# openshift/kubernetes-autoscaler

Hardware: NVIDIA B200
Metric: pod x node predicate evals/sec (higher is better)
Workload: dtype int64

## Files before the change

kubernetes-autoscaler_b200/csrc/api.cu:

```cuda
#include <algorithm>
#include <chrono>
#include <cstdio>
#include <cstdlib>
#include <cstring>
#include <map>
#include <tuple>
#include <unordered_map>

#include "engine.h"

namespace cae {

static thread_local std::string g_err;
void set_error(const std::string& msg) { g_err = msg; }

int Arena::alloc(void** dev, void** stage, size_t bytes) {
  bytes = (std::max<size_t>(bytes, 16) + 255) & ~(size_t)255;
  for (;;) {
    if (cur < chunks.size() && chunks[cur].used + bytes <= chunks[cur].size) break;
    if (cur + 1 < chunks.size()) { ++cur; continue; }
    Chunk c;
    c.size = std::max(bytes, min_chunk);
    if (cudaMalloc(&c.dev, c.size) != cudaSuccess) { set_error("cudaMalloc failed"); return -1; }
    if (mirrored && cudaHostAlloc(&c.host, c.size, cudaHostAllocDefault) != cudaSuccess) { set_error("cudaHostAlloc failed"); return -1; }
// ... 146 lines not shown
  UPV(dom, d.dom); UPV(dc_spec, d.dc_spec); UPV(dc_sc, d.dc_sc); UPV(dc_q_off, d.dc_q_off); UPV(q_kind, d.q_kind);
  UPV(q_k, d.q_k); UPV(q_dc, d.q_dc); UPV(q_p0, d.q_p0); UPV(q_base_off, d.q_base_off);
  UPV(spec_used, p8); e->d_spec_used = p8;
  UPV(dc_ngroups, p32); e->d_dc_ngroups = p32;
#undef UPV
  const size_t Q = std::max(d.Q, 1), pool = std::max(q_base_off.back(), 1);
  if (dev_alloc(e, &d.wmat, Q * S) || dev_alloc(e, &d.q_self, Q) || dev_alloc(e, &d.q_wown, Q) || dev_alloc(e, &d.q_active, Q) ||
      dev_alloc(e, &d.dc_aff_self, (size_t)d.DC) || dev_alloc(e, &d.dc_active, (size_t)d.DC) || dev_alloc(e, &d.elig, Q * e->U) ||
      dev_alloc(e, &d.base_cnt, pool, true) || dev_alloc(e, &d.base_pres, pool, true) || dev_alloc(e, &d.base_tot, Q, true) ||
      dev_alloc(e, &d.ds_w, Q * std::max(T, 1)) || dev_alloc(e, &d.st_min1, Q) || dev_alloc(e, &d.st_arg1, Q) ||
      dev_alloc(e, &d.st_min2, Q) || dev_alloc(e, &d.st_ndom, Q) || dev_alloc(e, &d.st_nmin, Q) || dev_alloc(e, &d.q_nfeed, Q, true) ||
      dev_alloc(e, &d.group_feeds, (size_t)std::max(e->E, 1), true) || dev_alloc(e, &d.qrec, Q))
    return -1;
  e->h_dc_of_spec_valid = true;
  return 0;
}

struct LoadTimer {
  bool on;
  std::chrono::steady_clock::time_point t0;
  std::string out;
  LoadTimer() : on(getenv("CAE_LOAD_TIMING") != nullptr), t0(std::chrono::steady_clock::now()) {}
  void mark(const char* what) {
    if (!on) return;
    auto t1 = std::chrono::steady_clock::now();
    char buf[96];
    snprintf(buf, sizeof(buf), " %s=%.1fus", what, std::chrono::duration<double, std::micro>(t1 - t0).count());
    out += buf;
    t0 = t1;
  }
  ~LoadTimer() { if (on) fprintf(stderr, "cae_load:%s\n", out.c_str()); }
};

static int stage_pending(Engine* e, int P, const int32_t* pend_spec, int E, const int32_t* group_off, bool check_pending) {
  const size_t words = (size_t)P + E + 1;
  if (words > e->pending_stage_words) {
    if (e->h_pending_stage) cudaFreeHost(e->h_pending_stage);
    e->h_pending_stage = nullptr;
    e->pending_stage_words = 0;
    const size_t cap_words = std::max(words, (size_t)e->cap_P + e->cap_E + 1);
    CAE_CUDA(cudaHostAlloc(reinterpret_cast<void**>(&e->h_pending_stage), cap_words * 4, cudaHostAllocDefault));
    e->pending_stage_words = cap_words;
  }
  const int S = e->num_podspecs;
  std::vector<int32_t> gspec(E, -1);
  bool homog = true;
  for (int g = 0; g < E; ++g) {
    const int b = group_off[g], en = group_off[g + 1];
    if (en <= b) continue;
    const int s0 = pend_spec[b];
    if (check_pending && (s0 < 0 || s0 >= S || !e->h_spec_pending[s0])) { set_error("cae_load_pending: a pod spec that was not pending at the last cae_load"); return 2; }
    gspec[g] = s0;
    int diff = 0;
    for (int p = b + 1; p < en; ++p) diff |= pend_spec[p] ^ s0;
    homog &= diff == 0;
  }
  if (!homog && check_pending)
    for (int p = 0; p < P; ++p) {
      const int s = pend_spec[p];
      if (s < 0 || s >= S || !e->h_spec_pending[s]) { set_error("cae_load_pending: a pod spec that was not pending at the last cae_load"); return 2; }
    }
  if (P) memcpy(e->h_pending_stage, pend_spec, sizeof(int32_t) * P);
  memcpy(e->h_pending_stage + P, group_off, sizeof(int32_t) * (E + 1));
  e->h_pend_spec = e->h_pending_stage;
  e->h_group_off = e->h_pending_stage + P;
  e->h_group_spec.swap(gspec);
  e->groups_homogeneous = homog;
  return 0;
}

static int do_load(Engine* e, const cae_objects* o) {
  LoadTimer lt;
  if (o->abi_version != CAE_ABI_VERSION) { set_error("cae_objects.abi_version mismatch"); return -2; }
  if (o->num_res < 3 || o->num_res > CAE_MAX_RES) { set_error("num_res out of range"); return 1; }
  e->up.reset();
  e->scratch.reset();
  e->loaded = false;
  e->group_reason_valid = false;
  e->stats.h2d_bytes = 0;
  const int N = o->num_cluster_nodes, T = o->num_templates, NT = N + T;
  e->N = N; e->T = T; e->U = N + 2 * T; e->E = o->num_groups; e->P = o->num_pending;
  e->Tw = (T + 31) / 32;
  e->Twp = (e->Tw + FEAS_TW - 1) / FEAS_TW * FEAS_TW;
  e->num_podspecs = o->num_podspecs;
  const int W = std::max(1, e->cfg.world_size), rk = e->cfg.rank;
  e->p_begin = (int)((int64_t)e->P * rk / W);
  e->p_end = (int)((int64_t)e->P * (rk + 1) / W);
  e->p_begin = (e->p_begin / 32) * 32;
  if (rk + 1 < W) e->p_end = (e->p_end / 32) * 32;
  if (e->cfg.flags & CAE_CFG_PODS_PRESHARDED) { e->p_begin = 0; e->p_end = e->P; }
  e->Pl = e->p_end - e->p_begin;
  e->Plw = (e->Pl + 31) / 32;
  e->t_begin = (int)((int64_t)T * rk / W);
  e->t_end = (int)((int64_t)T * (rk + 1) / W);

  cudaEventRecord(e->ev0, e->stream);
  DevObjects& d = e->dobj;
  d.num_res = o->num_res; d.num_values = o->num_values; d.hostname_key = o->hostname_key;
  d.unschedulable_taint_key = o->unschedulable_taint_key; d.N = N; d.T = T;
  UP(value_is_int, o->num_values); UP(value_int, o->num_values);
// ... 129 lines not shown
    }
  }
  e->feas_B = 0;
  e->feas_fstart = 0;
  for (int a = 0; a < e->A; ++a) {
    const int nb = f_bits[a] - 1;
    for (int i = nb - 1; i >= 0; --i) {
      if (e->feas_B >= 32) { set_error("resource request cardinality too large for the bit-sliced encoding"); return 1; }
      e->feas_sword[e->feas_B] = (uint8_t)f_word[a];
      e->feas_sshift[e->feas_B] = (uint8_t)(f_shift[a] + i);
      if (i == nb - 1) e->feas_fstart |= 1u << e->feas_B;
      ++e->feas_B;
    }
  }
  e->lut_rows = 0;
  for (int a = 0; a < e->A; ++a) {
    e->lut_base[a] = e->lut_rows;
    e->lut_rows += (int)rvals[a].size() + 1;
    e->lut_word[a] = (uint8_t)f_word[a];
    e->lut_shift[a] = (uint8_t)f_shift[a];
    e->lut_mask[a] = (1u << (f_bits[a] - 1)) - 1u;
  }
  e->d_tslice = nullptr;
  if (e->force_bitslice || e->lut_rows > FEAS_LUT_MAX_ROWS) {
    const int Bpad = std::max(4, (e->feas_B + 3) / 4 * 4);
    std::vector<uint32_t> tslice((size_t)Bpad * std::max(e->Tw, 1), 0);
    for (int b = 0; b < e->feas_B; ++b)
      for (int t = 0; t < T; ++t)
        tslice[(size_t)b * e->Tw + t / 32] |= ((tmpl_w[(size_t)e->feas_sword[b] * T + t] >> e->feas_sshift[b]) & 1u) << (t % 32);
    if (upload_mut(e, tslice, &e->d_tslice)) return -1;
  }
  {
    std::vector<uint32_t> rlut((size_t)std::max(e->lut_rows, 1) * std::max(e->Twp, 1), 0);
    for (int a = 0; a < e->A; ++a)
      for (int t = 0; t < T; ++t) {
        const uint32_t rank_free = (tmpl_w[(size_t)f_word[a] * T + t] >> f_shift[a]) & e->lut_mask[a];
        for (uint32_t k = 0; k <= rank_free; ++k) rlut[(size_t)(e->lut_base[a] + k) * e->Twp + t / 32] |= 1u << (t % 32);
      }
    if (upload_mut(e, rlut, &e->d_rlut)) return -1;
  }
  if (upload_mut(e, spec_sc, &e->d_spec_sc) || upload_mut(e, slots, &e->d_tmpl_slots) ||
      upload_mut(e, free_all, &e->d_tmpl_free_all) || upload_mut(e, free_act, &e->d_tmpl_free) || upload_mut(e, cfree, &e->d_c_free) ||
      upload_mut(e, cslots, &e->d_c_slots) || upload_mut(e, spec_w, &e->d_spec_w) || upload_mut(e, tmpl_w, &e->d_tmpl_w) || upload_mut(e, spec_dc, &e->d_spec_dc))
    return -1;

  lt.mark("ranks+tables");
  if (dev_alloc(e, &e->d_pre_ok, (size_t)e->SC * std::max(e->Twp, 1)) ||
      dev_alloc(e, &e->d_post_code, (size_t)e->DC * std::max(T, 1), true) || dev_alloc(e, &e->d_post_ok, (size_t)e->DC * std::max(e->Twp, 1)) ||
      dev_alloc(e, &e->d_pod_w, (size_t)std::max(e->W, 1) * std::max(e->Pl, 1)) || dev_alloc(e, &e->d_pod_row, (size_t)std::max(e->A, 1) * std::max(e->Pl, 1)) || dev_alloc(e, &e->d_pod_sc, (size_t)std::max(e->Pl, 1)) ||
      dev_alloc(e, &e->d_pod_dc, (size_t)std::max(e->Pl, 1)) || dev_alloc(e, &e->d_fit_bits, (size_t)std::max(T, 1) * std::max(e->Plw, 1)) ||
      dev_alloc(e, &e->d_fit_count, (size_t)std::max(T, 1), true) || dev_alloc(e, &e->d_fit_acc, (size_t)std::max(T, 1), true) ||
      dev_alloc(e, &e->d_chunk_done, (size_t)std::max(e->Twp / FEAS_TW, 1), true) || dev_alloc(e, &e->d_group_reason, (size_t)std::max(T, 1) * std::max(e->E, 1)) ||
      dev_alloc(e, &e->d_counts2, (size_t)2 * std::max(T, 1), true) || dev_alloc(e, &e->d_sched, (size_t)std::max(T, 1) * std::max(e->E, 1), true) ||
      dev_alloc(e, &e->d_order, (size_t)std::max(T, 1) * std::max(e->E, 1)) || dev_alloc(e, &e->d_grec, (size_t)std::max(e->E, 1)) || dev_alloc(e, &e->d_order_n, (size_t)std::max(T, 1), true) ||
      dev_alloc(e, &e->d_max_nodes, (size_t)std::max(T, 1), true) || dev_alloc(e, &e->d_last_index_buf, (size_t)2 * std::max(T, 1), true) || dev_alloc(e, &e->d_tmpl_cost, (size_t)std::max(T, 1), true) ||
      dev_alloc(e, &e->d_perm, (size_t)std::max(T, 1)) || dev_alloc(e, &e->d_work_counter, 4, true) ||
      dev_alloc(e, &e->d_act_dim, CAE_MAX_RES))
    return -1;
  e->d_score = nullptr;
  e->d_reasons = nullptr;
  if (e->cfg.want_reasons && dev_alloc(e, &e->d_reasons, (size_t)std::max(T, 1) * std::max(e->Pl, 1))) return -1;

  e->h_spec_pending = spec_pending;
  e->cap_P = e->P; e->cap_E = e->E; e->cap_Pl = e->Pl;
  { int rc = stage_pending(e, e->P, o->pend_spec, e->E, o->group_off, false); if (rc) return rc; }

  lt.mark("dev_alloc+memsets");
  if (e->up.flush(e->stream, &e->stats.h2d_bytes)) return -1;
  CAE_CUDA(cudaMemcpyAsync(e->d_act_dim, e->act_dim, sizeof(int) * CAE_MAX_RES, cudaMemcpyHostToDevice, e->stream));
  if (launch_pre_ok_bits(e)) return -1;
  if (e->has_dynamic) {
    if (launch_dynamic_tables(e, e->d_spec_used, e->d_dc_ngroups)) return -1;
    std::vector<uint8_t> act(e->dyn.DC);
    CAE_CUDA(cudaMemcpyAsync(act.data(), e->dyn.dc_active, act.size(), cudaMemcpyDeviceToHost, e->stream));
    CAE_CUDA(cudaStreamSynchronize(e->stream));
    bool changed = false;
    for (int s = 0; s < S; ++s) if (spec_dc[s] && !act[spec_dc[s]]) { spec_dc[s] = 0; changed = true; }
    if (changed) CAE_CUDA(cudaMemcpyAsync(e->d_spec_dc, spec_dc.data(), sizeof(int32_t) * S, cudaMemcpyHostToDevice, e->stream));
    e->h_spec_dc = spec_dc;
    CAE_CUDA(cudaStreamSynchronize(e->stream));
  }
  if (launch_post_bits(e)) return -1;
  if (launch_expand_pods(e)) return -1;
  if (launch_group_records(e)) return -1;
  cudaEventRecord(e->ev1, e->stream);
  lt.mark("launches");
  CAE_CUDA(cudaStreamSynchronize(e->stream));
  lt.mark("sync");
  float ms = 0;
  cudaEventElapsedTime(&ms, e->ev0, e->ev1);
  e->stats.h2d_ms = ms;
  e->loaded = true;
  return 0;
}

}

using cae::Engine;
// ... 107 lines not shown
  delete e;
}

int32_t cae_load(cae_engine* h, const cae_objects* objs) {
  if (!h || !objs) return -2;
  Engine* e = reinterpret_cast<Engine*>(h);
  cudaSetDevice(e->cfg.device);
  return cae::do_load(e, objs);
}

int32_t cae_load_pending(cae_engine* h, int32_t num_pending, const int32_t* pend_spec, int32_t num_groups, const int32_t* group_off) {
  Engine* e = reinterpret_cast<Engine*>(h);
  if (!e || !e->loaded) { cae::set_error("cae_load_pending before cae_load"); return -2; }
  if (num_pending < 0 || num_groups < 0 || (num_pending && !pend_spec) || !group_off) { cae::set_error("cae_load_pending: bad arguments"); return -2; }
  cudaSetDevice(e->cfg.device);
  const int P = num_pending, E = num_groups;
  const int W = std::max(1, e->cfg.world_size), rk = e->cfg.rank;
  int pb = (int)((int64_t)P * rk / W), pe = (int)((int64_t)P * (rk + 1) / W);
  pb = (pb / 32) * 32;
  if (rk + 1 < W) pe = (pe / 32) * 32;
  if (e->cfg.flags & CAE_CFG_PODS_PRESHARDED) { pb = 0; pe = P; }
  const int Pl = pe - pb;
  if (P > e->cap_P || E > e->cap_E || Pl > e->cap_Pl) { cae::set_error("cae_load_pending: more pods / groups than the resident buffers hold"); return 2; }
  if (group_off[0] != 0 || group_off[E] != P) { cae::set_error("cae_load_pending: group_off does not cover the pending pods"); return -2; }
  if (e->has_dynamic) {
    bool same = E == e->E;
    for (int g = 0; g < E && same; ++g) {
      const int s_new = group_off[g + 1] > group_off[g] ? pend_spec[group_off[g]] : -1;
      same = s_new == e->h_group_spec[g];
    }
    if (!same) { cae::set_error("cae_load_pending: the group -> spec sequence changed under topology counters"); return 2; }
  }
  CAE_CUDA(cudaStreamSynchronize(e->stream));
  { int rc = cae::stage_pending(e, P, pend_spec, E, group_off, true); if (rc) return rc; }
  const size_t words = (size_t)P + E + 1;
  if (P) CAE_CUDA(cudaMemcpyAsync(const_cast<int32_t*>(e->dobj.pend_spec), e->h_pend_spec, sizeof(int32_t) * P, cudaMemcpyHostToDevice, e->stream));
  CAE_CUDA(cudaMemcpyAsync(const_cast<int32_t*>(e->dobj.group_off), e->h_group_off, sizeof(int32_t) * (E + 1), cudaMemcpyHostToDevice, e->stream));
  e->stats.h2d_bytes = (int64_t)words * 4;
  e->P = P; e->E = E; e->p_begin = pb; e->p_end = pe; e->Pl = Pl; e->Plw = (Pl + 31) / 32;
  e->group_reason_valid = false;
  if (cae::launch_expand_pods(e)) return -1;
  if (cae::launch_group_records(e)) return -1;
  return 0;
}

int32_t cae_feasibility(cae_engine* h, uint32_t* fit_bits, uint8_t* reasons, int32_t* fit_count) {
  Engine* e = reinterpret_cast<Engine*>(h);
  if (!e || !e->loaded) { cae::set_error("cae_feasibility before cae_load"); return -2; }
  cudaSetDevice(e->cfg.device);
  bool want_r = e->cfg.want_reasons && e->d_reasons;
  cudaEventRecord(e->ev0, e->stream);
  if (cae::launch_feasibility(e, want_r)) return -1;
  cudaEventRecord(e->ev1, e->stream);
  e->stats.d2h_bytes = 0;
  if (!e->ev2) { cudaEventCreate(&e->ev2); cudaEventCreate(&e->ev3); }
  cudaEvent_t c0 = e->ev2, c1 = e->ev3;
  cudaEventRecord(c0, e->stream);
  if (fit_bits && e->T && e->Plw) {
    CAE_CUDA(cudaMemcpyAsync(fit_bits, e->d_fit_bits, sizeof(uint32_t) * (size_t)e->T * e->Plw, cudaMemcpyDeviceToHost, e->stream));
    e->stats.d2h_bytes += sizeof(uint32_t) * (size_t)e->T * e->Plw;
  }
  if (reasons && want_r && e->T && e->Pl) {
    CAE_CUDA(cudaMemcpyAsync(reasons, e->d_reasons, (size_t)e->T * e->Pl, cudaMemcpyDeviceToHost, e->stream));
    e->stats.d2h_bytes += (size_t)e->T * e->Pl;
  }
  if (fit_count && e->T) {
    CAE_CUDA(cudaMemcpyAsync(fit_count, e->d_fit_count, sizeof(int32_t) * e->T, cudaMemcpyDeviceToHost, e->stream));
// ... 515 lines not shown
```

kubernetes-autoscaler_b200/csrc/engine.h:

```cpp
#pragma once
#include <cuda_runtime.h>

#include <cstdint>
#include <string>
#include <vector>

#include "../../include/caengine.h"
#include "dyn.cuh"
#include "tables.cuh"

namespace cae {

constexpr int FEAS_MAX_W = 4;
constexpr int FEAS_LUT_MAX_ROWS = 1024;
constexpr int FEAS_TW = 16;

void set_error(const std::string& msg);

struct alignas(16) GroupRec {
  int32_t n, spec, sc, dc;
  uint32_t flags;
  int32_t pad[3];
  unsigned long long pconf, pbit;
  int64_t req[CAE_MAX_RES];
  float rinv[CAE_MAX_RES];
};
static_assert(sizeof(GroupRec) == 144, "GroupRec is fetched as nine 16-byte chunks");
enum : uint32_t { GREC_HAS_PORTS = 1u, GREC_FEEDS = 2u, GREC_HOST_SPREAD = 4u };
constexpr int ORDER_NOT_ON_FRESH = 1 << 30;

#define CAE_CUDA(expr)                                                                        \
  do {                                                                                        \
    cudaError_t _e = (expr);                                                                  \
    if (_e != cudaSuccess) {                                                                  \
      cae::set_error(std::string(#expr) + ": " + cudaGetErrorString(_e));                     \
      return -1;                                                                              \
    }                                                                                         \
  } while (0)

#define CAE_KERNEL_OK()                                                                       \
  do {                                                                                        \
    cudaError_t _e = cudaGetLastError();                                                      \
    if (_e != cudaSuccess) {                                                                  \
      cae::set_error(std::string(__func__) + ": " + cudaGetErrorString(_e));                  \
      return -1;                                                                              \
    }                                                                                         \
  } while (0)

// ... 31 lines not shown
  int A = 0;
  int act_dim[CAE_MAX_RES] = {0};
  int SC = 0, DC = 0;
  int Tw = 0;
  int Twp = 0;
  int p_begin = 0, p_end = 0;
  int t_begin = 0, t_end = 0;
  int Pl = 0, Plw = 0;
  bool has_dynamic = false;

  DevObjects dobj{};
  StaticClass* d_sclass = nullptr;
  uint8_t* d_pre_code = nullptr;
  uint32_t* d_pre_ok = nullptr;
  int32_t* d_spec_sc = nullptr;
  int32_t* d_spec_dc = nullptr;
  uint8_t* d_post_code = nullptr;
  uint32_t* d_post_ok = nullptr;
  int W = 0;
  uint32_t feas_guard[4] = {0, 0, 0, 0};
  uint32_t* d_spec_w = nullptr;
  uint32_t* d_pod_w = nullptr;
  uint16_t* d_pod_row = nullptr;
  uint32_t* d_tmpl_w = nullptr;
  int feas_B = 0;
  uint32_t feas_fstart = 0;
  uint8_t feas_sword[32] = {0}, feas_sshift[32] = {0};
  uint32_t* d_tslice = nullptr;
  int lut_rows = 0;
  int lut_base[CAE_MAX_RES] = {0};
  uint8_t lut_word[CAE_MAX_RES] = {0}, lut_shift[CAE_MAX_RES] = {0};
  uint32_t lut_mask[CAE_MAX_RES] = {0};
  uint32_t* d_rlut = nullptr;
  long long* d_tmpl_cost = nullptr;
  int32_t* d_perm = nullptr;
  int k1_warps = 16;
  bool force_bitslice = false;
  int32_t* d_pod_sc = nullptr;
  int32_t* d_pod_dc = nullptr;
  int64_t* d_tmpl_free = nullptr;
  int64_t* d_tmpl_free_all = nullptr;
  int32_t* d_tmpl_slots = nullptr;
  int64_t* d_spec_req_t = nullptr;
  uint32_t* d_fit_bits = nullptr;
  uint8_t* d_reasons = nullptr;
  int32_t* d_fit_count = nullptr;
  int32_t* d_fit_acc = nullptr;
  int32_t* d_chunk_done = nullptr;
  uint8_t* d_group_reason = nullptr;
  bool group_reason_valid = false;
  int32_t* d_counts2 = nullptr;
  int32_t* d_sched = nullptr;
  int32_t* d_order = nullptr;
  int32_t* d_order_n = nullptr;
  GroupRec* d_grec = nullptr;
  double* d_score = nullptr;
  int32_t* d_max_nodes = nullptr;
  int32_t* d_last_index_buf = nullptr;
  const int32_t* d_last_index_in = nullptr;
  int32_t* d_last_index_out = nullptr;
  int32_t* d_pc_of = nullptr;
  unsigned long long* d_port_conf = nullptr;
  int pack_cap = 1 << 30;
  void* d_pack_scratch = nullptr;
  size_t pack_scratch_bytes = 0;
  size_t pack_layout_sig = 0;
// ... 63 lines not shown
```

kubernetes-autoscaler_b200/csrc/feas.cu:

```cuda
#include <algorithm>
#include <climits>

#include "engine.h"

namespace cae {

struct LutLayout {
  int A, rows;
  int base[CAE_MAX_RES];
  uint32_t mask[CAE_MAX_RES];
  uint8_t word[CAE_MAX_RES], shift[CAE_MAX_RES];
};

static LutLayout lut_layout(const Engine* e) {
  LutLayout lay{};
  lay.A = e->A;
  lay.rows = e->lut_rows;
  for (int d = 0; d < e->A; ++d) {
    lay.base[d] = e->lut_base[d]; lay.mask[d] = e->lut_mask[d]; lay.word[d] = e->lut_word[d]; lay.shift[d] = e->lut_shift[d];
  }
  return lay;
}

__global__ void expand_pods_kernel(const int32_t* __restrict__ pend_spec, int p_begin, int Pl, int W, LutLayout lay,
// ... 10 lines not shown
  }
  pod_sc[p] = spec_sc[spec];
  pod_dc[p] = spec_dc[spec];
}

int launch_expand_pods(Engine* e) {
  if (e->Pl == 0) return 0;
  expand_pods_kernel<<<(e->Pl + 255) / 256, 256, 0, e->stream>>>(e->dobj.pend_spec, e->p_begin, e->Pl, e->W, lut_layout(e), e->d_spec_w,
                                                                   e->d_spec_sc, e->d_spec_dc, e->d_pod_w, e->d_pod_row, e->d_pod_sc, e->d_pod_dc);
  e->stats.kernel_launches++;
  CAE_KERNEL_OK();
  return 0;
}

constexpr int K1_TW = FEAS_TW;
constexpr int K1_TCHUNK = K1_TW * 32;
constexpr int K1_LPITCH = K1_TW + 1;

struct PeerPush {
  int world, rank;
  int tag;
  int2* data[8];
  int32_t* done_ctr;
  int32_t* status;
};

struct K1Args {
  int Pl, Plw, T, Tw, Twp, N, U, W;
  int G, gq, gr;
  const uint32_t* pod_w;
  const uint16_t* pod_row;
  const int32_t *pod_sc, *pod_dc;
  const uint32_t *tslice, *rlut;
  const int32_t* tmpl_slots;
  const uint32_t *pre_ok, *post_ok;
  const uint8_t *pre_code, *post_code;
  uint32_t* fit_bits;
  int32_t *fit_count, *fit_acc, *chunk_done;
  uint8_t* reasons;
};

__device__ __forceinline__ int k1_ld_acquire_sys(const int32_t* p) {
  int v;
  asm volatile("ld.acquire.sys.global.s32 %0, [%1];" : "=r"(v) : "l"(p) : "memory");
  return v;
}
__device__ __forceinline__ void k1_red_release_sys(int32_t* p, int v) {
  asm volatile("red.release.sys.global.add.s32 [%0], %1;" ::"l"(p), "r"(v) : "memory");
}
__device__ __forceinline__ void k1_st_volatile_v2(int2* p, int x, int y) {
  asm volatile("st.volatile.global.v2.s32 [%0], {%1, %2};" ::"l"(p), "r"(x), "r"(y) : "memory");
}
__device__ __forceinline__ int2 k1_ld_volatile_v2(const int2* p) {
  int2 v;
  asm volatile("ld.volatile.global.v2.s32 {%0, %1}, [%2];" : "=r"(v.x), "=r"(v.y) : "l"(p) : "memory");
  return v;
}
__device__ __forceinline__ unsigned long long k1_globaltimer() {
  unsigned long long t;
  asm volatile("mov.u64 %0, %%globaltimer;" : "=l"(t));
  return t;
}

__device__ __forceinline__ void k1_finish(const K1Args& a, const PeerPush& pp, const int32_t* s_cnt, int t0, int tid, int nthreads) {
  __shared__ int s_flag;
  for (int i = tid; i < K1_TCHUNK; i += nthreads) {
    const int c = s_cnt[i];
    if (c && t0 + i < a.T) atomicAdd(&a.fit_acc[t0 + i], c);
  }
  __syncthreads();
  if (tid == 0) {
    __threadfence();
    s_flag = atomicAdd(&a.chunk_done[blockIdx.y], 1) == (int)gridDim.x - 1;
  }
  __syncthreads();
  if (!s_flag) return;
  __threadfence();
  for (int i = tid; i < K1_TCHUNK; i += nthreads) {
    const int t = t0 + i;
    if (t < a.T) {
      a.fit_count[t] = __ldcg(&a.fit_acc[t]);
      a.fit_acc[t] = 0;
    }
  }
  if (tid == 0) a.chunk_done[blockIdx.y] = 0;
  if (!pp.world) return;
  __syncthreads();
  if (tid == 0) {
    __threadfence();
    s_flag = atomicAdd(pp.done_ctr, 1) == (int)gridDim.y - 1;
  }
  __syncthreads();
  if (!s_flag) return;
  __threadfence();
  const int tag = pp.tag;
  for (int r = 0; r < pp.world; ++r) {
    int2* dst = pp.data[r] + (size_t)pp.rank * Engine::PEER_CAP;
    for (int t = tid; t < a.T; t += nthreads) k1_st_volatile_v2(dst + t, __ldcg(&a.fit_count[t]), tag);
  }
  const int2* mine = pp.data[pp.rank];
  const unsigned long long t0ns = k1_globaltimer();
  int ok = 1;
  for (int t = tid; t < a.T && ok; t += nthreads) {
    int2 x[Engine::PEER_MAX];
    unsigned pending = 0;
#pragma unroll
    for (int r = 0; r < Engine::PEER_MAX; ++r)
      if (r < pp.world) x[r] = k1_ld_volatile_v2(mine + (size_t)r * Engine::PEER_CAP + t);
#pragma unroll
    for (int r = 0; r < Engine::PEER_MAX; ++r)
      if (r < pp.world && x[r].y != tag) pending |= 1u << r;
    for (int spins = 0; pending; ) {
#pragma unroll
      for (int r = 0; r < Engine::PEER_MAX; ++r)
        if ((pending >> r) & 1u) {
          x[r] = k1_ld_volatile_v2(mine + (size_t)r * Engine::PEER_CAP + t);
          if (x[r].y == tag) pending &= ~(1u << r);
        }
      if (pending && (++spins & 1023) == 0 && k1_globaltimer() - t0ns > 2000000000ull) { ok = 0; break; }
    }
    int v = 0;
#pragma unroll
    for (int r = 0; r < Engine::PEER_MAX; ++r)
      if (r < pp.world) v += x[r].x;
    if (ok) a.fit_count[t] = v;
  }
  if (!ok) atomicExch(pp.status, 1);
  if (tid == 0) *pp.done_ctr = 0;
}

struct TransposeConsts { uint32_t sel16, sel8, amt[3], keep[3]; };

__device__ __forceinline__ uint32_t opaque(uint32_t v) {
  uint32_t r;
  asm volatile("mov.b32 %0, %1;" : "=r"(r) : "r"(v));
  return r;
}

__device__ __forceinline__ TransposeConsts transpose_consts(int lane) {
  TransposeConsts c;
  c.sel16 = opaque((lane & 16) ? 0x3276u : 0x5410u);
  c.sel8 = opaque((lane & 8) ? 0x3715u : 0x6240u);
#pragma unroll
  for (int i = 0; i < 3; ++i) {
    const int s = 4 >> i;
    const uint32_t lowmask = s == 4 ? 0x0F0F0F0Fu : s == 2 ? 0x33333333u : 0x55555555u;
    c.amt[i] = opaque((lane & s) ? (uint32_t)s : (uint32_t)(32 - s));
    c.keep[i] = opaque((lane & s) ? ~lowmask : lowmask);
  }
  return c;
}

__device__ __forceinline__ uint32_t bitselect(uint32_t x, uint32_t y, uint32_t keep) {
  uint32_t r;
  asm("lop3.b32 %0, %1, %2, %3, 0xE4;" : "=r"(r) : "r"(x), "r"(y), "r"(keep));
  return r;
}

__device__ __forceinline__ void warp_transpose32x2(uint32_t& a, uint32_t& b, const TransposeConsts& c) {
  uint32_t ya = __shfl_xor_sync(0xffffffffu, a, 16), yb = __shfl_xor_sync(0xffffffffu, b, 16);
  a = __byte_perm(a, ya, c.sel16);
// ... 82 lines not shown
        const int wglob = tw0 + tw + h;
        const uint32_t fit = h ? fit1 : fit0;
        if (valid && wglob < a.Tw) {
          for (int j = 0; j < 32; ++j) {
            const int t = wglob * 32 + j;
            if (t >= a.T) break;
            uint8_t rs = a.pre_code[(size_t)sc * a.U + a.N + t] & 0x0F;
            if (rs == 0) rs = (!((fit >> j) & 1u) || a.tmpl_slots[t] < 1) ? CAE_R_FIT : a.post_code[(size_t)dc * a.T + t];
            a.reasons[(size_t)t * a.Pl + p] = rs;
          }
        }
      }
    }
    uint32_t c0 = fit0 & cls[tw], c1 = fit1 & cls[tw + 1];
    warp_transpose32x2(c0, c1, tc);
    s_out[warp * PAD + tw * 32 + lane] = c0;
    s_out[warp * PAD + (tw + 1) * 32 + lane] = c1;
    atomicAdd(&s_cnt[tw * 32 + lane], __popc(c0));
    atomicAdd(&s_cnt[(tw + 1) * 32 + lane], __popc(c1));
  }
  __syncthreads();
  if (a.fit_bits) {
    const int wv = tid % NW;
    if (wv < npw) {
      uint32_t* dst = a.fit_bits + (size_t)(t0 + tid / NW) * a.Plw + pwb + wv;
      const uint32_t* src = s_out + wv * PAD + tid / NW;
      const size_t stride = (size_t)32 * a.Plw;
      const int kmax = min(K1_TCHUNK / 32, (a.T - t0 - tid / NW + 31) / 32);
#pragma unroll 4
      for (int k = 0; k < kmax; ++k, dst += stride, src += 32) *dst = *src;
    }
  }
  k1_finish(a, pp, s_cnt, t0, tid, NT);
}

constexpr int K1_THREADS = 256;
constexpr int K1_WARPS = K1_THREADS / 32;
constexpr int K1_PAD = K1_TCHUNK + 4;

struct FeasLayout {
  uint32_t fstart;
  int nb;
  uint8_t sword[32], sshift[32];
};

template <int B, bool REASONS>
__global__ void __launch_bounds__(K1_THREADS)
feasibility_kernel(K1Args a, FeasLayout lay, PeerPush pp) {
  __shared__ uint32_t s_sl[B > 0 ? B : 1][K1_TW];
  __shared__ uint32_t s_out[K1_WARPS][K1_PAD];
  __shared__ int32_t s_cnt[K1_TCHUNK];
  const int tid = threadIdx.x, lane = tid & 31, warp = tid >> 5;
  const int p = blockIdx.x * K1_THREADS + tid;
  const int tw0 = blockIdx.y * K1_TW;
  const int t0 = tw0 * 32;

  for (int i = tid; i < B * K1_TW; i += K1_THREADS) {
    const int b = i / K1_TW, w = i % K1_TW;
    s_sl[b][w] = (tw0 + w < a.Tw) ? a.tslice[(size_t)b * a.Tw + tw0 + w] : 0u;
  }
  for (int i = tid; i < K1_TCHUNK; i += K1_THREADS) s_cnt[i] = 0;
  const bool valid = p < a.Pl;
  uint32_t r[B > 0 ? B : 1];
  {
    uint32_t pw[FEAS_MAX_W];
#pragma unroll
// ... 40 lines not shown
  }
  __syncthreads();
  const int pw0 = blockIdx.x * K1_WARPS;
  for (int i = tid; i < K1_TCHUNK * K1_WARPS; i += K1_THREADS) {
    const int tl = i / K1_WARPS, wv = i % K1_WARPS;
    const int t = t0 + tl;
    if (t < a.T && pw0 + wv < a.Plw && a.fit_bits) a.fit_bits[(size_t)t * a.Plw + pw0 + wv] = s_out[wv][tl];
  }
  k1_finish(a, pp, s_cnt, t0, tid, K1_THREADS);
}

static PeerPush peer_push_args(Engine* e) {
  PeerPush pp{};
  if (e->peer_world > 1 && e->T <= Engine::PEER_CAP) {
    const int par = (int)(e->peer_step & 1);
    const size_t blk = (size_t)Engine::PEER_MAX * Engine::PEER_CAP;
    pp.world = e->peer_world;
    pp.rank = e->cfg.rank;
    e->peer_step += 1;
    pp.tag = (int)(e->peer_step & 0x7fffffff);
    if (pp.tag == 0) pp.tag = 1;
    for (int r = 0; r < e->peer_world; ++r) pp.data[r] = reinterpret_cast<int2*>(e->peer_base[r]) + par * blk;
    pp.done_ctr = e->d_xbuf + 4 * blk + 8;
    pp.status = e->d_xbuf + 4 * blk + 9;
  }
  return pp;
}

static K1Args k1_args(Engine* e) {
  K1Args a{};
  a.Pl = e->Pl; a.Plw = e->Plw; a.T = e->T; a.Tw = e->Tw; a.Twp = e->Twp; a.N = e->N; a.U = e->U; a.W = e->W;
  a.G = 1;
  a.pod_w = e->d_pod_w; a.pod_row = e->d_pod_row; a.pod_sc = e->d_pod_sc; a.pod_dc = e->d_pod_dc;
  a.tslice = e->d_tslice; a.rlut = e->d_rlut; a.tmpl_slots = e->d_tmpl_slots;
  a.pre_ok = e->d_pre_ok; a.post_ok = e->d_post_ok; a.pre_code = e->d_pre_code; a.post_code = e->d_post_code;
  a.fit_bits = e->d_fit_bits; a.fit_count = e->d_fit_count; a.fit_acc = e->d_fit_acc; a.chunk_done = e->d_chunk_done;
  a.reasons = e->d_reasons;
  return a;
}

template <int B>
static void launch_feas_b(Engine* e, bool want_reasons, K1Args a, const PeerPush& pp) {
  dim3 grid((e->Pl + K1_THREADS - 1) / K1_THREADS, e->Twp / K1_TW);
  FeasLayout lay;
  lay.fstart = e->feas_fstart;
  lay.nb = e->feas_B;
  for (int b = 0; b < 32; ++b) { lay.sword[b] = e->feas_sword[b]; lay.sshift[b] = e->feas_sshift[b]; }
  if (want_reasons) feasibility_kernel<B, true><<<grid, K1_THREADS, 0, e->stream>>>(a, lay, pp);
  else feasibility_kernel<B, false><<<grid, K1_THREADS, 0, e->stream>>>(a, lay, pp);
}

template <int A, bool REASONS, int NW>
static int launch_feas_lut_arw(Engine* e, K1Args a, const PeerPush& pp) {
  const int chunks = e->Twp / K1_TW;
  const int slots = e->sm_count * (48 / NW);
  const int g_min = (e->Plw + NW - 1) / NW;
  a.G = std::max(g_min, std::min(e->Plw, std::max(1, slots / chunks)));
  a.gq = e->Plw / a.G;
  a.gr = e->Plw % a.G;
  dim3 grid(a.G, chunks);
  const size_t smem = sizeof(uint32_t) * ((size_t)std::max(e->lut_rows, 1) * K1_LPITCH + NW * (K1_TCHUNK + 32 / NW) + K1_TCHUNK);
  auto kern = feasibility_lut_kernel<A, REASONS, NW>;
  if (smem > 48 * 1024) CAE_CUDA(cudaFuncSetAttribute(kern, cudaFuncAttributeMaxDynamicSharedMemorySize, (int)smem));
  kern<<<grid, NW * 32, smem, e->stream>>>(a, e->lut_rows, pp);
  return 0;
}

template <int A>
static int launch_feas_lut_a(Engine* e, bool want_reasons, const K1Args& a, const PeerPush& pp) {
  if (e->k1_warps == 8)
    return want_reasons ? launch_feas_lut_arw<A, true, 8>(e, a, pp) : launch_feas_lut_arw<A, false, 8>(e, a, pp);
  return want_reasons ? launch_feas_lut_arw<A, true, 16>(e, a, pp) : launch_feas_lut_arw<A, false, 16>(e, a, pp);
}

constexpr int K1_LUT_MAX_ROWS = FEAS_LUT_MAX_ROWS;

int launch_feasibility(Engine* e, bool want_reasons) {
  if (e->Tw == 0) return 0;
  if (e->Pl == 0) {
    CAE_CUDA(cudaMemsetAsync(e->d_fit_count, 0, sizeof(int32_t) * e->T, e->stream));
    return 0;
  }
  if (e->peer_world > 1 && e->T > Engine::PEER_CAP) {
    set_error("fused histogram exchange: more templates than the exchange buffer holds (use the NCCL all-reduce of cae_device_buffer(0))");
    return 1;
  }
  const PeerPush pp = peer_push_args(e);
  const K1Args a = k1_args(e);
  if (!e->force_bitslice && e->lut_rows <= K1_LUT_MAX_ROWS) {
    int rc = 0;
    switch (e->A) {
      case 0: rc = launch_feas_lut_a<0>(e, want_reasons, a, pp); break;
      case 1: rc = launch_feas_lut_a<1>(e, want_reasons, a, pp); break;
      case 2: rc = launch_feas_lut_a<2>(e, want_reasons, a, pp); break;
      case 3: rc = launch_feas_lut_a<3>(e, want_reasons, a, pp); break;
      case 4: rc = launch_feas_lut_a<4>(e, want_reasons, a, pp); break;
      case 5: rc = launch_feas_lut_a<5>(e, want_reasons, a, pp); break;
      case 6: rc = launch_feas_lut_a<6>(e, want_reasons, a, pp); break;
      case 7: rc = launch_feas_lut_a<7>(e, want_reasons, a, pp); break;
      default: rc = launch_feas_lut_a<8>(e, want_reasons, a, pp); break;
    }
    if (rc) return rc;
  } else {
    const int Bp = e->feas_B == 0 ? 0 : (e->feas_B + 3) / 4 * 4;
    switch (Bp) {
      case 0: launch_feas_b<0>(e, want_reasons, a, pp); break;
      case 4: launch_feas_b<4>(e, want_reasons, a, pp); break;
      case 8: launch_feas_b<8>(e, want_reasons, a, pp); break;
      case 12: launch_feas_b<12>(e, want_reasons, a, pp); break;
      case 16: launch_feas_b<16>(e, want_reasons, a, pp); break;
      case 20: launch_feas_b<20>(e, want_reasons, a, pp); break;
      case 24: launch_feas_b<24>(e, want_reasons, a, pp); break;
      case 28: launch_feas_b<28>(e, want_reasons, a, pp); break;
      default: launch_feas_b<32>(e, want_reasons, a, pp); break;
    }
  }
  e->stats.kernel_launches++;
  CAE_KERNEL_OK();
  return 0;
}

}
```

Measured before the change: 5740 billion.

## Add template-major feasibility kernel using per-pod threshold masks and class-run detection

```diff
diff --git a/kubernetes-autoscaler_b200/csrc/api.cu b/kubernetes-autoscaler_b200/csrc/api.cu
--- a/kubernetes-autoscaler_b200/csrc/api.cu
+++ b/kubernetes-autoscaler_b200/csrc/api.cu
@@ -202,7 +202,7 @@
   ~LoadTimer() { if (on) fprintf(stderr, "cae_load:%s\n", out.c_str()); }
 };
 
-static int stage_pending(Engine* e, int P, const int32_t* pend_spec, int E, const int32_t* group_off, bool check_pending) {
+static int stage_pending(Engine* e, int P, const int32_t* pend_spec, int E, const int32_t* group_off, bool check_pending, int pb, int pe) {
   const size_t words = (size_t)P + E + 1;
   if (words > e->pending_stage_words) {
     if (e->h_pending_stage) cudaFreeHost(e->h_pending_stage);
@@ -215,6 +215,10 @@
   const int S = e->num_podspecs;
   std::vector<int32_t> gspec(E, -1);
   bool homog = true;
+  std::vector<uint8_t> wruns((size_t)(std::max(pe - pb, 0) + 31) / 32, 1);
+  auto spec_change = [&](int p) {
+    if (p > pb && p < pe && ((p - pb) & 31) && pend_spec[p] != pend_spec[p - 1]) ++wruns[(p - pb) >> 5];
+  };
   for (int g = 0; g < E; ++g) {
     const int b = group_off[g], en = group_off[g + 1];
     if (en <= b) continue;
@@ -224,18 +228,24 @@
     int diff = 0;
     for (int p = b + 1; p < en; ++p) diff |= pend_spec[p] ^ s0;
     homog &= diff == 0;
+    spec_change(b);
+    if (diff)
+      for (int p = b + 1; p < en; ++p) spec_change(p);
   }
   if (!homog && check_pending)
     for (int p = 0; p < P; ++p) {
       const int s = pend_spec[p];
       if (s < 0 || s >= S || !e->h_spec_pending[s]) { set_error("cae_load_pending: a pod spec that was not pending at the last cae_load"); return 2; }
     }
+  int runs_max = 0;
+  for (uint8_t r : wruns) runs_max = std::max(runs_max, (int)r);
   if (P) memcpy(e->h_pending_stage, pend_spec, sizeof(int32_t) * P);
   memcpy(e->h_pending_stage + P, group_off, sizeof(int32_t) * (E + 1));
   e->h_pend_spec = e->h_pending_stage;
   e->h_group_off = e->h_pending_stage + P;
   e->h_group_spec.swap(gspec);
   e->groups_homogeneous = homog;
+  e->pod_runs_max = runs_max;
   return 0;
 }
 
@@ -431,12 +441,17 @@
   }
   {
     std::vector<uint32_t> rlut((size_t)std::max(e->lut_rows, 1) * std::max(e->Twp, 1), 0);
-    for (int a = 0; a < e->A; ++a)
+    const size_t tp = (size_t)e->Twp * 32;
+    std::vector<uint16_t> trow((size_t)A1 * std::max(tp, (size_t)1), 0);
+    for (int a = 0; a < e->A; ++a) {
+      for (size_t t = T; t < tp; ++t) trow[a * tp + t] = (uint16_t)e->lut_base[a];
       for (int t = 0; t < T; ++t) {
         const uint32_t rank_free = (tmpl_w[(size_t)f_word[a] * T + t] >> f_shift[a]) & e->lut_mask[a];
         for (uint32_t k = 0; k <= rank_free; ++k) rlut[(size_t)(e->lut_base[a] + k) * e->Twp + t / 32] |= 1u << (t % 32);
+        trow[a * tp + t] = (uint16_t)std::min<uint32_t>(e->lut_base[a] + rank_free, 0xFFFF);
       }
-    if (upload_mut(e, rlut, &e->d_rlut)) return -1;
+    }
+    if (upload_mut(e, rlut, &e->d_rlut) || upload_mut(e, trow, &e->d_tmpl_row)) return -1;
   }
   if (upload_mut(e, spec_sc, &e->d_spec_sc) || upload_mut(e, slots, &e->d_tmpl_slots) ||
       upload_mut(e, free_all, &e->d_tmpl_free_all) || upload_mut(e, free_act, &e->d_tmpl_free) || upload_mut(e, cfree, &e->d_c_free) ||
@@ -449,7 +464,7 @@
       dev_alloc(e, &e->d_pod_w, (size_t)std::max(e->W, 1) * std::max(e->Pl, 1)) || dev_alloc(e, &e->d_pod_row, (size_t)std::max(e->A, 1) * std::max(e->Pl, 1)) || dev_alloc(e, &e->d_pod_sc, (size_t)std::max(e->Pl, 1)) ||
       dev_alloc(e, &e->d_pod_dc, (size_t)std::max(e->Pl, 1)) || dev_alloc(e, &e->d_fit_bits, (size_t)std::max(T, 1) * std::max(e->Plw, 1)) ||
       dev_alloc(e, &e->d_fit_count, (size_t)std::max(T, 1), true) || dev_alloc(e, &e->d_fit_acc, (size_t)std::max(T, 1), true) ||
-      dev_alloc(e, &e->d_chunk_done, (size_t)std::max(e->Twp / FEAS_TW, 1), true) || dev_alloc(e, &e->d_group_reason, (size_t)std::max(T, 1) * std::max(e->E, 1)) ||
+      dev_alloc(e, &e->d_chunk_done, (size_t)std::max(e->Twp / FEAS_TMAJ_TW, 1), true) || dev_alloc(e, &e->d_group_reason, (size_t)std::max(T, 1) * std::max(e->E, 1)) ||
       dev_alloc(e, &e->d_counts2, (size_t)2 * std::max(T, 1), true) || dev_alloc(e, &e->d_sched, (size_t)std::max(T, 1) * std::max(e->E, 1), true) ||
       dev_alloc(e, &e->d_order, (size_t)std::max(T, 1) * std::max(e->E, 1)) || dev_alloc(e, &e->d_grec, (size_t)std::max(e->E, 1)) || dev_alloc(e, &e->d_order_n, (size_t)std::max(T, 1), true) ||
       dev_alloc(e, &e->d_max_nodes, (size_t)std::max(T, 1), true) || dev_alloc(e, &e->d_last_index_buf, (size_t)2 * std::max(T, 1), true) || dev_alloc(e, &e->d_tmpl_cost, (size_t)std::max(T, 1), true) ||
@@ -462,7 +477,7 @@
 
   e->h_spec_pending = spec_pending;
   e->cap_P = e->P; e->cap_E = e->E; e->cap_Pl = e->Pl;
-  { int rc = stage_pending(e, e->P, o->pend_spec, e->E, o->group_off, false); if (rc) return rc; }
+  { int rc = stage_pending(e, e->P, o->pend_spec, e->E, o->group_off, false, e->p_begin, e->p_end); if (rc) return rc; }
 
   lt.mark("dev_alloc+memsets");
   if (e->up.flush(e->stream, &e->stats.h2d_bytes)) return -1;
@@ -636,7 +651,7 @@
     if (!same) { cae::set_error("cae_load_pending: the group -> spec sequence changed under topology counters"); return 2; }
   }
   CAE_CUDA(cudaStreamSynchronize(e->stream));
-  { int rc = cae::stage_pending(e, P, pend_spec, E, group_off, true); if (rc) return rc; }
+  { int rc = cae::stage_pending(e, P, pend_spec, E, group_off, true, pb, pe); if (rc) return rc; }
   const size_t words = (size_t)P + E + 1;
   if (P) CAE_CUDA(cudaMemcpyAsync(const_cast<int32_t*>(e->dobj.pend_spec), e->h_pend_spec, sizeof(int32_t) * P, cudaMemcpyHostToDevice, e->stream));
   CAE_CUDA(cudaMemcpyAsync(const_cast<int32_t*>(e->dobj.group_off), e->h_group_off, sizeof(int32_t) * (E + 1), cudaMemcpyHostToDevice, e->stream));
diff --git a/kubernetes-autoscaler_b200/csrc/engine.h b/kubernetes-autoscaler_b200/csrc/engine.h
--- a/kubernetes-autoscaler_b200/csrc/engine.h
+++ b/kubernetes-autoscaler_b200/csrc/engine.h
@@ -14,6 +14,11 @@
 constexpr int FEAS_MAX_W = 4;
 constexpr int FEAS_LUT_MAX_ROWS = 1024;
 constexpr int FEAS_TW = 16;
+constexpr int FEAS_TMAJ_TW = 8;
+#ifndef CAE_TMAJ_MAX_RUNS
+#define CAE_TMAJ_MAX_RUNS 8
+#endif
+constexpr int FEAS_TMAJ_MAX_RUNS = CAE_TMAJ_MAX_RUNS;
 
 void set_error(const std::string& msg);
 
@@ -111,6 +116,8 @@
   uint8_t lut_word[CAE_MAX_RES] = {0}, lut_shift[CAE_MAX_RES] = {0};
   uint32_t lut_mask[CAE_MAX_RES] = {0};
   uint32_t* d_rlut = nullptr;
+  uint16_t* d_tmpl_row = nullptr;
+  int pod_runs_max = 0;
   long long* d_tmpl_cost = nullptr;
   int32_t* d_perm = nullptr;
   int k1_warps = 16;
diff --git a/kubernetes-autoscaler_b200/csrc/feas.cu b/kubernetes-autoscaler_b200/csrc/feas.cu
--- a/kubernetes-autoscaler_b200/csrc/feas.cu
+++ b/kubernetes-autoscaler_b200/csrc/feas.cu
@@ -66,6 +66,7 @@
   const uint16_t* pod_row;
   const int32_t *pod_sc, *pod_dc;
   const uint32_t *tslice, *rlut;
+  const uint16_t* tmpl_row;
   const int32_t* tmpl_slots;
   const uint32_t *pre_ok, *post_ok;
   const uint8_t *pre_code, *post_code;
@@ -96,12 +97,9 @@
   return t;
 }
 
-__device__ __forceinline__ void k1_finish(const K1Args& a, const PeerPush& pp, const int32_t* s_cnt, int t0, int tid, int nthreads) {
+template <int TCHUNK>
+__device__ __forceinline__ void k1_publish(const K1Args& a, const PeerPush& pp, int t0, int tid, int nthreads) {
   __shared__ int s_flag;
-  for (int i = tid; i < K1_TCHUNK; i += nthreads) {
-    const int c = s_cnt[i];
-    if (c && t0 + i < a.T) atomicAdd(&a.fit_acc[t0 + i], c);
-  }
   __syncthreads();
   if (tid == 0) {
     __threadfence();
@@ -110,7 +108,7 @@
   __syncthreads();
   if (!s_flag) return;
   __threadfence();
-  for (int i = tid; i < K1_TCHUNK; i += nthreads) {
+  for (int i = tid; i < TCHUNK; i += nthreads) {
     const int t = t0 + i;
     if (t < a.T) {
       a.fit_count[t] = __ldcg(&a.fit_acc[t]);
@@ -161,6 +159,14 @@
   }
   if (!ok) atomicExch(pp.status, 1);
   if (tid == 0) *pp.done_ctr = 0;
+}
+
+__device__ __forceinline__ void k1_finish(const K1Args& a, const PeerPush& pp, const int32_t* s_cnt, int t0, int tid, int nthreads) {
+  for (int i = tid; i < K1_TCHUNK; i += nthreads) {
+    const int c = s_cnt[i];
+    if (c && t0 + i < a.T) atomicAdd(&a.fit_acc[t0 + i], c);
+  }
+  k1_publish<K1_TCHUNK>(a, pp, t0, tid, nthreads);
 }
 
 struct TransposeConsts { uint32_t sel16, sel8, amt[3], keep[3]; };
@@ -309,6 +315,146 @@
     }
   }
   k1_finish(a, pp, s_cnt, t0, tid, NT);
+}
+
+constexpr int TM_NW = FEAS_TMAJ_TW;
+constexpr int TM_TCHUNK = TM_NW * 32;
+constexpr int TM_PW = 32;
+constexpr int TM_WPW = TM_PW / TM_NW;
+constexpr int TM_CPITCH = TM_PW + 1;
+static_assert(FEAS_TW % TM_NW == 0 && TM_NW % 4 == 0, "chunks of the template-major pass tile the row pitch Twp; 128-bit class loads");
+
+struct TmajLayout {
+  int rows, mp;
+  int base[CAE_MAX_RES + 1];
+};
+
+template <int A>
+__global__ void __launch_bounds__(TM_NW * 32, 3)
+feasibility_tmaj_kernel(K1Args a, TmajLayout lay, PeerPush pp) {
+  extern __shared__ uint32_t k1_smem[];
+  constexpr int TRW = A > 4 ? 4 : 2;
+  uint32_t* s_m = k1_smem;
+  uint32_t* s_cw = s_m + TM_PW * lay.mp;
+  uint32_t* s_tr = s_cw + TM_NW * TM_PW * TM_CPITCH;
+  __shared__ uint32_t s_lead[TM_PW], s_valid[TM_PW];
+  const int lane = threadIdx.x & 31, warp = threadIdx.x >> 5;
+  const int tw0 = blockIdx.y * TM_NW;
+  const int tw = tw0 + warp;
+  const int pw0 = blockIdx.x * TM_PW;
+
+  int prow[TM_WPW][A > 0 ? A : 1], sc[TM_WPW], dc[TM_WPW];
+#pragma unroll
+  for (int k = 0; k < TM_WPW; ++k) {
+    const int p = (pw0 + warp + k * TM_NW) * 32 + lane;
+    const bool valid = p < a.Pl;
+#pragma unroll
+    for (int d = 0; d < A; ++d) prow[k][d] = valid ? (int)a.pod_row[(size_t)d * a.Pl + p] : INT_MAX;
+    sc[k] = valid ? a.pod_sc[p] : -1;
+    dc[k] = valid ? a.pod_dc[p] : 0;
+  }
+  uint32_t tr[A > 0 ? A : 1];
+#pragma unroll
+  for (int d = 0; d < A; ++d) tr[d] = a.tmpl_row[(size_t)d * a.Twp * 32 + tw * 32 + lane];
+  uint32_t cw[TM_WPW][TM_NW];
+#pragma unroll
+  for (int k = 0; k < TM_WPW; ++k) {
+    const uint4* pre = reinterpret_cast<const uint4*>(a.pre_ok + (size_t)max(sc[k], 0) * a.Twp + tw0);
+    const uint4* post = reinterpret_cast<const uint4*>(a.post_ok + (size_t)dc[k] * a.Twp + tw0);
+#pragma unroll
+    for (int q = 0; q < TM_NW / 4; ++q) {
+      uint4 u = make_uint4(0, 0, 0, 0);
+      if (sc[k] >= 0) {
+        const uint4 x = __ldg(pre + q), y = __ldg(post + q);
+        u = make_uint4(x.x & y.x, x.y & y.y, x.z & y.z, x.w & y.w);
+      }
+      cw[k][4 * q + 0] = u.x; cw[k][4 * q + 1] = u.y; cw[k][4 * q + 2] = u.z; cw[k][4 * q + 3] = u.w;
+    }
+  }
+#pragma unroll
+  for (int k = 0; k < TM_WPW; ++k) {
+    const int w = warp + k * TM_NW;
+    const int psc = __shfl_up_sync(0xffffffffu, sc[k], 1), pdc = __shfl_up_sync(0xffffffffu, dc[k], 1);
+    const uint32_t lead = __ballot_sync(0xffffffffu, sc[k] >= 0 && (lane == 0 || psc != sc[k] || pdc != dc[k]));
+    const uint32_t valid = __ballot_sync(0xffffffffu, sc[k] >= 0);
+    if (lane == 0) { s_lead[w] = lead; s_valid[w] = valid; }
+#pragma unroll
+    for (int i = 0; i < TM_NW; ++i) s_cw[(i * TM_PW + w) * TM_CPITCH + lane] = cw[k][i];
+  }
+  {
+    uint32_t keep[TM_WPW];
+#pragma unroll
+    for (int k = 0; k < TM_WPW; ++k) keep[k] = 0;
+    int r = 0;
+#pragma unroll
+    for (int d = 0; d < A; ++d) {
+#pragma unroll 1
+      for (; r < lay.base[d + 1]; ++r) {
+#pragma unroll
+        for (int k = 0; k < TM_WPW; ++k) {
+          const uint32_t b = __ballot_sync(0xffffffffu, prow[k][d] <= r);
+          if (lane == (r & 31)) keep[k] = b;
+        }
+        if ((r & 31) == 31) {
+#pragma unroll
+          for (int k = 0; k < TM_WPW; ++k) s_m[(warp + k * TM_NW) * lay.mp + r - 31 + lane] = keep[k];
+        }
+      }
+    }
+    if (lane < (lay.rows & 31)) {
+#pragma unroll
+      for (int k = 0; k < TM_WPW; ++k) s_m[(warp + k * TM_NW) * lay.mp + (lay.rows & ~31) + lane] = keep[k];
+    }
+  }
+  if constexpr (A > 0) {
+    uint32_t x[TRW];
+#pragma unroll
+    for (int i = 0; i < TRW; ++i) x[i] = (2 * i < A ? tr[min(2 * i, A - 1)] : 0u) | (2 * i + 1 < A ? tr[min(2 * i + 1, A - 1)] << 16 : 0u);
+    if constexpr (TRW == 4) reinterpret_cast<uint4*>(s_tr)[warp * 32 + lane] = make_uint4(x[0], x[1], x[TRW > 2 ? 2 : 0], x[TRW > 3 ? 3 : 0]);
+    else reinterpret_cast<uint2*>(s_tr)[warp * 32 + lane] = make_uint2(x[0], x[1]);
+  }
+  __syncthreads();
+
+  const uint32_t lead = s_lead[lane], vmask = s_valid[lane];
+  const uint32_t* cwp = s_cw + (warp * TM_PW + lane) * TM_CPITCH;
+  uint32_t cm[32];
+#pragma unroll
+  for (int j = 0; j < 32; ++j) cm[j] = 0;
+  for (uint32_t rest = lead; rest;) {
+    const int i = __ffs(rest) - 1;
+    rest &= rest - 1;
+    const uint32_t run = (rest ? (rest & (0u - rest)) - 1u : 0xffffffffu) & ~((1u << i) - 1u) & vmask;
+    const uint32_t c = cwp[i];
+#pragma unroll
+    for (int j = 0; j < 32; ++j) cm[j] |= run & (0u - ((c >> j) & 1u));
+  }
+
+  const int wg = pw0 + lane;
+  const bool store = a.fit_bits != nullptr && wg < a.Plw;
+  const uint32_t* mrow = s_m + lane * lay.mp;
+  int cnt = 0;
+#pragma unroll
+  for (int j = 0; j < 32; ++j) {
+    uint32_t f = cm[j];
+    if constexpr (A > 0) {
+      uint32_t x[TRW];
+      if constexpr (TRW == 4) {
+        const uint4 v = reinterpret_cast<const uint4*>(s_tr)[warp * 32 + j];
+        x[0] = v.x; x[1] = v.y; x[TRW > 2 ? 2 : 0] = v.z; x[TRW > 3 ? 3 : 0] = v.w;
+      } else {
+        const uint2 v = reinterpret_cast<const uint2*>(s_tr)[warp * 32 + j];
+        x[0] = v.x; x[1] = v.y;
+      }
+#pragma unroll
+      for (int d = 0; d < A; ++d) f &= mrow[(x[d >> 1] >> (16 * (d & 1))) & 0xFFFFu];
+    }
+    const int t = tw * 32 + j;
+    if (store && t < a.T) a.fit_bits[(size_t)t * a.Plw + wg] = f;
+    const int c = (int)__reduce_add_sync(0xffffffffu, (unsigned)__popc(f));
+    cnt = lane == j ? c : cnt;
+  }
+  if (cnt && tw * 32 + lane < a.T) atomicAdd(&a.fit_acc[tw * 32 + lane], cnt);
+  k1_publish<TM_TCHUNK>(a, pp, tw0 * 32, threadIdx.x, TM_NW * 32);
 }
 
 constexpr int K1_THREADS = 256;
@@ -415,7 +561,7 @@
   a.Pl = e->Pl; a.Plw = e->Plw; a.T = e->T; a.Tw = e->Tw; a.Twp = e->Twp; a.N = e->N; a.U = e->U; a.W = e->W;
   a.G = 1;
   a.pod_w = e->d_pod_w; a.pod_row = e->d_pod_row; a.pod_sc = e->d_pod_sc; a.pod_dc = e->d_pod_dc;
-  a.tslice = e->d_tslice; a.rlut = e->d_rlut; a.tmpl_slots = e->d_tmpl_slots;
+  a.tslice = e->d_tslice; a.rlut = e->d_rlut; a.tmpl_row = e->d_tmpl_row; a.tmpl_slots = e->d_tmpl_slots;
   a.pre_ok = e->d_pre_ok; a.post_ok = e->d_post_ok; a.pre_code = e->d_pre_code; a.post_code = e->d_post_code;
   a.fit_bits = e->d_fit_bits; a.fit_count = e->d_fit_count; a.fit_acc = e->d_fit_acc; a.chunk_done = e->d_chunk_done;
   a.reasons = e->d_reasons;
@@ -458,6 +604,29 @@
 
 constexpr int K1_LUT_MAX_ROWS = FEAS_LUT_MAX_ROWS;
 
+template <int A>
+static int launch_feas_tmaj_a(Engine* e, const K1Args& a, const PeerPush& pp) {
+  TmajLayout lay{};
+  lay.rows = e->lut_rows;
+  lay.mp = e->lut_rows | 1;
+  for (int d = 0; d < A; ++d) lay.base[d] = e->lut_base[d];
+  lay.base[A] = e->lut_rows;
+  dim3 grid((e->Plw + TM_PW - 1) / TM_PW, e->Twp / TM_NW);
+  constexpr int TRW = A > 4 ? 4 : 2;
+  const size_t smem = sizeof(uint32_t) * ((size_t)TM_PW * lay.mp + TM_NW * TM_PW * TM_CPITCH + TM_TCHUNK * TRW);
+  if (smem > (size_t)e->smem_optin) { set_error("dense pass: threshold masks exceed the shared memory of a thread block"); return -1; }
+  auto kern = feasibility_tmaj_kernel<A>;
+  if (smem > 48 * 1024) CAE_CUDA(cudaFuncSetAttribute(kern, cudaFuncAttributeMaxDynamicSharedMemorySize, (int)smem));
+  kern<<<grid, TM_NW * 32, smem, e->stream>>>(a, lay, pp);
+  return 0;
+}
+
+template <int A>
+static int launch_feas_fast_a(Engine* e, bool want_reasons, const K1Args& a, const PeerPush& pp) {
+  if (!want_reasons && e->pod_runs_max <= FEAS_TMAJ_MAX_RUNS) return launch_feas_tmaj_a<A>(e, a, pp);
+  return launch_feas_lut_a<A>(e, want_reasons, a, pp);
+}
+
 int launch_feasibility(Engine* e, bool want_reasons) {
   if (e->Tw == 0) return 0;
   if (e->Pl == 0) {
@@ -473,15 +642,15 @@
   if (!e->force_bitslice && e->lut_rows <= K1_LUT_MAX_ROWS) {
     int rc = 0;
     switch (e->A) {
-      case 0: rc = launch_feas_lut_a<0>(e, want_reasons, a, pp); break;
-      case 1: rc = launch_feas_lut_a<1>(e, want_reasons, a, pp); break;
-      case 2: rc = launch_feas_lut_a<2>(e, want_reasons, a, pp); break;
-      case 3: rc = launch_feas_lut_a<3>(e, want_reasons, a, pp); break;
-      case 4: rc = launch_feas_lut_a<4>(e, want_reasons, a, pp); break;
-      case 5: rc = launch_feas_lut_a<5>(e, want_reasons, a, pp); break;
-      case 6: rc = launch_feas_lut_a<6>(e, want_reasons, a, pp); break;
-      case 7: rc = launch_feas_lut_a<7>(e, want_reasons, a, pp); break;
-      default: rc = launch_feas_lut_a<8>(e, want_reasons, a, pp); break;
+      case 0: rc = launch_feas_fast_a<0>(e, want_reasons, a, pp); break;
+      case 1: rc = launch_feas_fast_a<1>(e, want_reasons, a, pp); break;
+      case 2: rc = launch_feas_fast_a<2>(e, want_reasons, a, pp); break;
+      case 3: rc = launch_feas_fast_a<3>(e, want_reasons, a, pp); break;
+      case 4: rc = launch_feas_fast_a<4>(e, want_reasons, a, pp); break;
+      case 5: rc = launch_feas_fast_a<5>(e, want_reasons, a, pp); break;
+      case 6: rc = launch_feas_fast_a<6>(e, want_reasons, a, pp); break;
+      case 7: rc = launch_feas_fast_a<7>(e, want_reasons, a, pp); break;
+      default: rc = launch_feas_fast_a<8>(e, want_reasons, a, pp); break;
     }
     if (rc) return rc;
   } else {
```

New measurement: 4835 billion, median of 6. 0.842x the previous value.
